# dibbelab/gficf

Hardware: AMD Instinct MI355X
Metric: jaccard_edges_per_sec (higher is better)
Workload: dtype int32

## Files before the change

### gficf_amd/csrc/knn.hip

```cpp
#include <cfloat>
#include <cstdlib>
#include <cstring>
#include <vector>

#include "common.h"
#include "knn_tiles.h"

namespace {

constexpr int KNN_MAX_D = 128;
constexpr int KNN_MAX_SPLIT = 16;

__host__ __device__ inline int knn_dpad(int d) { return (d + 3) & ~3; }

template <typename T>
__global__ __launch_bounds__(256) void k_knn_prepare(const T* __restrict__ X, int64_t n_rows, int d, int dpad, int64_t ld,
                                                     int metric, float* __restrict__ out, uint32_t* __restrict__ status) {
  const int64_t r = (int64_t)blockIdx.x * 256 + threadIdx.x;
  if (r >= n_rows) return;
  bool bad = false;
  float inv = 1.0f;
  bool scale = false;
  float mean = 0.0f;
  if (metric == GFICF_KNN_CORRELATION) {
// ... 71 lines not shown
  const int64_t e = (int64_t)blockIdx.x * 256 + threadIdx.x;
  if (e < n) v[e] = (int32_t)e;
}

constexpr int KNN_CELL_KEY_BITS = 20;
__global__ __launch_bounds__(256) void k_knn_sort_elems(const int32_t* __restrict__ pivot_of, const int32_t* __restrict__ coarse_of,
                                                        int64_t n, u64* __restrict__ kv) {
  const int64_t e = (int64_t)blockIdx.x * 256 + threadIdx.x;
  if (e < n) {
    const int32_t f = pivot_of[e];
    kv[e] = ((u64)(uint32_t)(((coarse_of[f - 1] - 1) << 12) | (f - 1)) << 32) | (u64)e;
  }
}

template <int METRIC>
__device__ inline float knn_bound_dist(const float* __restrict__ a, const float* __restrict__ b, int d) {
  float acc = 0.0f;
  for (int t = 0; t < d; ++t) {
    const float df = a[t] - b[t];
    acc = METRIC == GFICF_KNN_MANHATTAN ? acc + fabsf(df) : fmaf(df, df, acc);
  }
  return METRIC == GFICF_KNN_MANHATTAN ? acc : sqrtf(acc);
}

template <int METRIC>
__global__ __launch_bounds__(KNN_TC) void k_knn_tile_stats(const float* __restrict__ X, const int32_t* __restrict__ tile_n, int d, int dpad,
                                                           float* __restrict__ centers, float* __restrict__ radius) {
  __shared__ float s_c[KNN_MAX_D];
  __shared__ float s_r[KNN_TC / 64];
  const int64_t t = blockIdx.x, j0 = t * KNN_TC;
  const int n = tile_n[t];
  if (n <= 0) { if (threadIdx.x == 0) radius[t] = -1.0f; return; }
  for (int dim = threadIdx.x; dim < dpad; dim += KNN_TC) {
    float sum = 0.0f;
    for (int p = 0; p < n; ++p) sum += X[(j0 + p) * dpad + dim];
    const float c = sum / (float)n;
    s_c[dim] = c;
    centers[(int64_t)dim * gridDim.x + t] = c;
  }
  __syncthreads();
  float r = 0.0f;
  if ((int)threadIdx.x < n) r = knn_bound_dist<METRIC>(X + (j0 + threadIdx.x) * dpad, s_c, d);
#pragma unroll
  for (int w = 32; w >= 1; w >>= 1) r = fmaxf(r, __shfl_xor(r, w));
  if ((threadIdx.x & 63) == 0) s_r[threadIdx.x >> 6] = r;
  __syncthreads();
  if (threadIdx.x == 0) radius[t] = fmaxf(s_r[0], s_r[1]);
}

template <int METRIC>
__global__ __launch_bounds__(256) void k_knn_lb(const float* __restrict__ Q, const int32_t* __restrict__ qtile_n, int d, int dpad,
                                                const float* __restrict__ centers, const float* __restrict__ radius,
                                                const int32_t* __restrict__ tile_n, int kk, int64_t n_ct, float* __restrict__ lb,
                                                unsigned long long* __restrict__ counters) {
  extern __shared__ __attribute__((aligned(16))) float s_q[];
  __shared__ float s_u[4];
  const int64_t qt = blockIdx.x, q0 = qt * KNN_TQ;
  const int nq = qtile_n[qt];
  if (nq <= 0) return;
  for (int e = threadIdx.x; e < KNN_TQ * dpad; e += 256) {
    const int row = e / dpad, dim = e % dpad;
    s_q[dim * KNN_TQ + row] = row < nq ? Q[(q0 + row) * dpad + dim] : 0.0f;
  }
  __syncthreads();
  const int lane = threadIdx.x & 63, wave = threadIdx.x >> 6;
  const float key_abs_slack = (float)(d + 8) * 1.1920929e-7f;
  auto to_key = [key_abs_slack](float e, float slack_sign) {
    if (METRIC == GFICF_KNN_MANHATTAN) return e;
    if (METRIC == GFICF_KNN_EUCLIDEAN) return e * e * (1.0f + slack_sign * KNN_LB_SLACK);
    return 0.5f * e * e * (1.0f + slack_sign * KNN_LB_SLACK) + slack_sign * key_abs_slack;
  };
  float u = INFINITY;
  for (int64_t c = threadIdx.x; c < n_ct; c += 256) {
    const float r = radius[c];
    if (r < 0.0f) { lb[qt * n_ct + c] = INFINITY; continue; }
    float mn = INFINITY, mx = 0.0f;
    for (int g0 = 0; g0 < nq; g0 += 16) {
      float acc[16];
#pragma unroll
      for (int j = 0; j < 16; ++j) acc[j] = 0.0f;
      for (int t = 0; t < d; ++t) {
        const float cv = centers[(int64_t)t * n_ct + c];
        const float4* q4 = reinterpret_cast<const float4*>(s_q + t * KNN_TQ + g0);
#pragma unroll
        for (int j4 = 0; j4 < 4; ++j4) {
          const float4 q = q4[j4];
          const float qa[4] = {q.x, q.y, q.z, q.w};
#pragma unroll
          for (int j = 0; j < 4; ++j) {
            const float df = qa[j] - cv;
            acc[4 * j4 + j] = METRIC == GFICF_KNN_MANHATTAN ? acc[4 * j4 + j] + fabsf(df) : fmaf(df, df, acc[4 * j4 + j]);
          }
        }
      }
#pragma unroll
      for (int j = 0; j < 16; ++j) {
        if (g0 + j < nq) {
          const float e = METRIC == GFICF_KNN_MANHATTAN ? acc[j] : sqrtf(acc[j]);
          mn = fminf(mn, e); mx = fmaxf(mx, e);
        }
      }
    }
    float b = mn - r - KNN_LB_SLACK * (mn + r);
    b = b > 0.0f ? to_key(b, -1.0f) : 0.0f;
    lb[qt * n_ct + c] = b > 0.0f ? b : 0.0f;
    if (tile_n[c] >= kk) u = fminf(u, to_key((mx + r) * (1.0f + KNN_LB_SLACK), 1.0f));
  }
#pragma unroll
  for (int w = 32; w >= 1; w >>= 1) u = fminf(u, __shfl_xor(u, w));
  if (lane == 0) s_u[wave] = u;
  __syncthreads();
  const float U = fminf(fminf(s_u[0], s_u[1]), fminf(s_u[2], s_u[3]));
  int npr = 0, np = 0;
  for (int64_t c = threadIdx.x; c < n_ct; c += 256) {
    const float b = lb[qt * n_ct + c];
    if (b < INFINITY) { ++np; npr += b > U ? 1 : 0; }
  }
#pragma unroll
  for (int w = 32; w >= 1; w >>= 1) { npr += __shfl_xor(npr, w); np += __shfl_xor(np, w); }
  if (lane == 0) { atomicAdd(counters, (unsigned long long)npr); atomicAdd(counters + 1, (unsigned long long)np); }
}

__global__ void k_knn_choose(const unsigned long long* __restrict__ counters, uint32_t force, uint32_t* __restrict__ flag) {
  *flag = force ? 0u : (2ull * counters[0] < counters[1] ? 1u : 0u);
}

__global__ __launch_bounds__(256) void k_knn_cell_heads(const int32_t* __restrict__ keys, int64_t n, int64_t* __restrict__ flags) {
  const int64_t p = (int64_t)blockIdx.x * 256 + threadIdx.x;
  if (p > n) return;
  flags[p] = (p < n && (p == 0 || keys[p] != keys[p - 1])) ? 1 : 0;
}
__global__ __launch_bounds__(256) void k_knn_cell_starts(const int32_t* __restrict__ keys, const int64_t* __restrict__ rank, int64_t n,
                                                         int32_t* __restrict__ cstart) {
  const int64_t p = (int64_t)blockIdx.x * 256 + threadIdx.x;
  if (p > n) return;
  if (p == n) { cstart[rank[n]] = (int32_t)n; return; }
  if (p == 0 || keys[p] != keys[p - 1]) cstart[rank[p]] = (int32_t)p;
}
__global__ __launch_bounds__(1024) void k_knn_cell_offsets(const int32_t* __restrict__ cstart, const int64_t* __restrict__ n_cells_p, int T,
                                                           int32_t* __restrict__ pstart) {
  __shared__ int s_part[1024];
  __shared__ int s_total;
  const int n_cells = (int)*n_cells_p;
  const int per = (n_cells + 1023) / 1024;
  const int c0 = threadIdx.x * per;
  int sum = 0;
  for (int c = c0; c < c0 + per && c < n_cells; ++c) sum += (cstart[c + 1] - cstart[c] + T - 1) / T * T;
  s_part[threadIdx.x] = sum;
  __syncthreads();
  if (threadIdx.x == 0) {
    int run = 0;
    for (int t = 0; t < 1024; ++t) { const int v = s_part[t]; s_part[t] = run; run += v; }
    s_total = run;
  }
  __syncthreads();
  int run = s_part[threadIdx.x];
  for (int c = c0; c < c0 + per && c < n_cells; ++c) { pstart[c] = run; run += (cstart[c + 1] - cstart[c] + T - 1) / T * T; }
  if (threadIdx.x == 0) pstart[n_cells] = s_total;
}
__global__ __launch_bounds__(256) void k_knn_pad_scatter(const int32_t* __restrict__ keys, const int64_t* __restrict__ rank,
                                                         const int32_t* __restrict__ cstart, const int32_t* __restrict__ pstart,
                                                         const int32_t* __restrict__ perm, int64_t n, int nq4,
                                                         const float* __restrict__ src, float* __restrict__ dst, int32_t* __restrict__ perm_pad) {
  const int64_t e = (int64_t)blockIdx.x * 256 + threadIdx.x;
  if (e >= n * nq4) return;
  const int64_t p = e / nq4;
  const int q4 = (int)(e % nq4);
  const bool head = p == 0 || keys[p] != keys[p - 1];
  const int64_t c = rank[p] + (head ? 1 : 0) - 1;
  const int64_t pp = (int64_t)pstart[c] + (p - cstart[c]);
  const int32_t id = perm[p];
  reinterpret_cast<float4*>(dst)[pp * nq4 + q4] = reinterpret_cast<const float4*>(src)[(int64_t)id * nq4 + q4];
  if (q4 == 0) perm_pad[pp] = id;
// ... 1 lines not shown
__global__ __launch_bounds__(256) void k_knn_tile_counts(const int32_t* __restrict__ perm_pad, int64_t n_tiles, int T, int32_t* __restrict__ tile_n) {
  const int64_t t = (int64_t)blockIdx.x * 256 + threadIdx.x;
  if (t >= n_tiles) return;
  int n = 0;
  for (int r = 0; r < T; ++r) n += perm_pad[t * T + r] >= 0 ? 1 : 0;
  tile_n[t] = n;
}

int knn_split(const gficf_ctx* ctx, int64_t n_q, int64_t N) {
  const int64_t n_qt = gficf_ceil_div(n_q > 0 ? n_q : 1, KNN_TQ), n_ct = gficf_ceil_div(N > 0 ? N : 1, KNN_TC);
  int64_t S = gficf_ceil_div((int64_t)ctx->num_cus * 8, n_qt);
  if (S > n_ct / 8) S = n_ct / 8;
  if (S > KNN_MAX_SPLIT) S = KNN_MAX_SPLIT;
  if (S < 1) S = 1;
  if (const char* e = getenv("GFICF_KNN_SPLIT")) {
    const int v = atoi(e);
    if (v >= 1 && v <= KNN_MAX_SPLIT) S = v;
  }
  return (int)S;
}

constexpr int64_t KNN_PRUNE_MIN_N = 30000;
constexpr int64_t KNN_PRUNE_MAX_TILES = 8192;
bool knn_use_prune(int64_t N) {
  const int64_t n_ct = gficf_ceil_div(N > 0 ? N : 1, KNN_TC);
  if (n_ct < 2 || n_ct > KNN_PRUNE_MAX_TILES) return false;
  if (const char* e = getenv("GFICF_KNN_PRUNE")) return atoi(e) != 0;
  return N >= KNN_PRUNE_MIN_N;
}
inline int64_t knn_coarse(int64_t C) { return C / 16 > 2 ? C / 16 : 2; }

int64_t knn_pivots(int64_t N) {
  int64_t per = 256;
  if (const char* e = getenv("GFICF_KNN_PIVOT_CELL")) per = atoi(e) > 0 ? atoi(e) : per;
  int64_t c = gficf_ceil_div(N, per);
  return c < 2 ? 2 : c > 4096 ? 4096 : c;
}

int knn_check(int64_t N, int d, int k, int metric) {
  if (N < 0 || d < 0 || k < 0) GFICF_FAIL(GFICF_ERR_INVALID_ARG, "negative size");
  if (N > 0x7FFFFFFFll) GFICF_FAIL(GFICF_ERR_UNSUPPORTED, "N = %lld exceeds int32 ids", (long long)N);
  if (d > KNN_MAX_D) GFICF_FAIL(GFICF_ERR_UNSUPPORTED, "d = %d exceeds %d dimensions", d, KNN_MAX_D);
  if (k > GFICF_KNN_MAX_K) GFICF_FAIL(GFICF_ERR_UNSUPPORTED, "k = %d exceeds GFICF_KNN_MAX_K = %d", k, GFICF_KNN_MAX_K);
  if (k > N) GFICF_FAIL(GFICF_ERR_INVALID_ARG, "k = %d neighbours asked of N = %lld points", k, (long long)N);
  if (!gficf_knn_metric_ok(metric)) GFICF_FAIL(GFICF_ERR_INVALID_ARG, "unknown metric %d", metric);
  return GFICF_OK;
}

struct KnnPruneWs {
  int64_t C, xrows, qrows, n_ct, n_qt;
  float *pivots, *coarse, *xp, *qp, *centers, *radius, *lb;
  u64* apart;
  int32_t *pivot_of, *coarse_of, *key_tmp, *perm_sorted, *perm_x, *perm_q, *cstart, *pstart, *tile_n, *qtile_n;
  int64_t* rank;
  u64 *kv0, *kv1;
  int64_t* hist;
  u64* part;
  u64* part_plain;
  unsigned long long* counters;
  size_t total;
};

KnnPruneWs knn_prune_ws(char* base, int64_t n_q, int64_t N, int dpad, int k) {
  KnnPruneWs w{};
  gficf_carver cv{base};
  const int64_t C = knn_pivots(N);
  w.C = C;
  w.n_ct = gficf_ceil_div(N, KNN_TC) + (C < N ? C : N);
  w.n_qt = gficf_ceil_div(n_q, KNN_TQ) + (C < n_q ? C : n_q);
  w.xrows = w.n_ct * KNN_TC;
  w.qrows = w.n_qt * KNN_TQ;
  w.pivots = cv.take<float>((size_t)C * dpad);
  w.coarse = cv.take<float>((size_t)knn_coarse(C) * dpad);
  w.coarse_of = cv.take<int32_t>((size_t)C);
  w.xp = cv.take<float>((size_t)w.xrows * dpad);
  w.qp = cv.take<float>((size_t)w.qrows * dpad);
  w.centers = cv.take<float>((size_t)w.n_ct * dpad);
  w.radius = cv.take<float>((size_t)w.n_ct);
  w.lb = cv.take<float>((size_t)w.n_qt * w.n_ct);
  w.apart = cv.take<u64>((size_t)N);
  w.pivot_of = cv.take<int32_t>((size_t)N);
  w.key_tmp = cv.take<int32_t>((size_t)N);
  w.perm_sorted = cv.take<int32_t>((size_t)N);
  w.perm_x = cv.take<int32_t>((size_t)w.xrows);
  w.perm_q = cv.take<int32_t>((size_t)w.qrows);
  w.cstart = cv.take<int32_t>((size_t)(C + 2));
  w.pstart = cv.take<int32_t>((size_t)(C + 2));
  w.tile_n = cv.take<int32_t>((size_t)w.n_ct);
  w.qtile_n = cv.take<int32_t>((size_t)w.n_qt);
  w.rank = cv.take<int64_t>((size_t)(N + 1));
  w.kv0 = cv.take<u64>((size_t)N);
  w.kv1 = cv.take<u64>((size_t)N);
  w.hist = cv.take<int64_t>((size_t)gficf_radix_sort_hist_len(N, KNN_CELL_KEY_BITS));
  w.part = cv.take<u64>((size_t)w.qrows * (size_t)k);
  w.part_plain = cv.take<u64>((size_t)n_q * (size_t)KNN_MAX_SPLIT * (size_t)k);
  w.counters = cv.take<unsigned long long>(4);
  w.total = cv.total();
  return w;
}

}

extern "C" {

int gficf_knn_dpad(int d) { return (d < 0 || d > KNN_MAX_D) ? -1 : knn_dpad(d); }

int gficf_knn_prepare_device(gficf_ctx* ctx, const void* d_X, int x_is_f64, int64_t n_rows, int d, int64_t ld, int metric,
                             float* d_point_rows) {
  GFICF_CTX_ENTER(ctx);
  int rc = knn_check(n_rows, d, 0, metric);
  if (rc) return rc;
  if (n_rows == 0 || d == 0) return GFICF_OK;
  if (!d_X || !d_point_rows) GFICF_FAIL(GFICF_ERR_INVALID_ARG, "NULL device pointer");
  if (ld < n_rows) GFICF_FAIL(GFICF_ERR_INVALID_ARG, "ld = %lld < n_rows = %lld", (long long)ld, (long long)n_rows);
  const unsigned blocks = (unsigned)gficf_ceil_div(n_rows, 256);
  if (x_is_f64)
    hipLaunchKernelGGL(k_knn_prepare<double>, dim3(blocks), dim3(256), 0, ctx->stream, (const double*)d_X, n_rows, d, knn_dpad(d), ld, metric, d_point_rows, ctx->d_status);
  else
    hipLaunchKernelGGL(k_knn_prepare<float>, dim3(blocks), dim3(256), 0, ctx->stream, (const float*)d_X, n_rows, d, knn_dpad(d), ld, metric, d_point_rows, ctx->d_status);
  GFICF_HIP_CHECK(hipGetLastError());
  return GFICF_OK;
}

size_t gficf_knn_workspace_bytes(gficf_ctx* ctx, int64_t n_queries, int64_t N, int k) {
  if (!ctx || n_queries <= 0 || N <= 0 || k <= 0) return 256;
  const size_t plain = (size_t)n_queries * (size_t)KNN_MAX_SPLIT * (size_t)k * sizeof(u64) + 256;
  const size_t small = (size_t)n_queries * (size_t)knn_split(ctx, n_queries, N) * (size_t)k * sizeof(u64) + 256;
  const size_t pruned = gficf_ceil_div(N, KNN_TC) <= KNN_PRUNE_MAX_TILES ? knn_prune_ws(nullptr, n_queries, N, knn_dpad(KNN_MAX_D), k).total : 0;
  (void)plain;
  return small > pruned ? small : pruned;
}

int gficf_knn_search_device(gficf_ctx* ctx, const float* d_points, int64_t N, int d, int k, int metric, int64_t q_begin,
                            int64_t q_end, void* d_ws, size_t ws_bytes, int32_t* d_idx, float* d_dist, int64_t ld_out) {
  GFICF_CTX_ENTER(ctx);
  int rc = knn_check(N, d, k, metric);
  if (rc) return rc;
  if (q_begin < 0 || q_end < q_begin || q_end > N)
    GFICF_FAIL(GFICF_ERR_INVALID_ARG, "query range [%lld, %lld) outside [0, %lld]", (long long)q_begin, (long long)q_end, (long long)N);
  const int64_t n_q = q_end - q_begin;
  if (n_q == 0 || k == 0) return GFICF_OK;
  if (d == 0) GFICF_FAIL(GFICF_ERR_INVALID_ARG, "points have no dimensions");
  if (!d_points || !d_ws || !d_idx) GFICF_FAIL(GFICF_ERR_INVALID_ARG, "NULL device pointer");
  if (ld_out < n_q) GFICF_FAIL(GFICF_ERR_INVALID_ARG, "ld_out = %lld < number of queries %lld", (long long)ld_out, (long long)n_q);
  if (ws_bytes < gficf_knn_workspace_bytes(ctx, n_q, N, k)) GFICF_FAIL(GFICF_ERR_CAPACITY, "kNN workspace too small");
  metric = gficf_knn_search_metric(metric);
  const int dpad = knn_dpad(d);
  const unsigned mblocks = (unsigned)gficf_ceil_div(n_q, 256);
  KnnTileArgs a{};
  a.d = d; a.dpad = dpad; a.kk = k;

  if (!knn_use_prune(N)) {
    a.Q = d_points + q_begin * dpad; a.n_q = n_q; a.X = d_points; a.N = N;
    a.S = knn_split(ctx, n_q, N);
    a.part = (u64*)d_ws;
    rc = knn_launch_m<false>(ctx, metric, a);
    if (rc) return rc;
    hipLaunchKernelGGL(k_knn_merge, dim3(mblocks), dim3(256), 0, ctx->stream, a.part, n_q, a.S, k, metric, (const int32_t*)nullptr, d_idx, d_dist, ld_out, (const uint32_t*)nullptr, 0u);
    GFICF_HIP_CHECK(hipGetLastError());
    return GFICF_OK;
  }

  const KnnPruneWs w = knn_prune_ws((char*)d_ws, n_q, N, dpad, k);
  const int nq4 = dpad >> 2;
  const int64_t C = w.C;
  auto blocks_for = [](int64_t n) { return dim3((unsigned)gficf_ceil_div(n, 256)); };
  hipLaunchKernelGGL(k_knn_gather_rows, blocks_for(C * nq4), dim3(256), 0, ctx->stream, d_points, (const int32_t*)nullptr, C, nq4, N / C, w.pivots);
  KnnTileArgs as{};
  as.Q = d_points; as.n_q = N; as.X = w.pivots; as.N = C; as.d = d; as.dpad = dpad; as.kk = 1; as.S = 1; as.part = w.apart;
  rc = knn_launch_m<false>(ctx, metric, as);
  if (rc) return rc;
  hipLaunchKernelGGL(k_knn_merge, blocks_for(N), dim3(256), 0, ctx->stream, w.apart, N, 1, 1, metric, (const int32_t*)nullptr, w.pivot_of, (float*)nullptr, N, (const uint32_t*)nullptr, 0u);
  const int64_t Cc = knn_coarse(C);
  hipLaunchKernelGGL(k_knn_gather_rows, blocks_for(Cc * nq4), dim3(256), 0, ctx->stream, w.pivots, (const int32_t*)nullptr, Cc, nq4, C / Cc, w.coarse);
  KnnTileArgs ac{};
  ac.Q = w.pivots; ac.n_q = C; ac.X = w.coarse; ac.N = Cc; ac.d = d; ac.dpad = dpad; ac.kk = 1; ac.S = 1; ac.part = w.apart;
  rc = knn_launch_m<false>(ctx, metric, ac);
  if (rc) return rc;
  hipLaunchKernelGGL(k_knn_merge, blocks_for(C), dim3(256), 0, ctx->stream, w.apart, C, 1, 1, metric, (const int32_t*)nullptr, w.coarse_of, (float*)nullptr, C, (const uint32_t*)nullptr, 0u);
  GFICF_HIP_CHECK(hipMemsetAsync(w.xp, 0, sizeof(float) * (size_t)w.xrows * dpad, ctx->stream));
  GFICF_HIP_CHECK(hipMemsetAsync(w.qp, 0, sizeof(float) * (size_t)w.qrows * dpad, ctx->stream));
  GFICF_HIP_CHECK(hipMemsetAsync(w.perm_x, 0xFF, sizeof(int32_t) * (size_t)w.xrows, ctx->stream));
  GFICF_HIP_CHECK(hipMemsetAsync(w.perm_q, 0xFF, sizeof(int32_t) * (size_t)w.qrows, ctx->stream));
  auto layout = [&](int64_t first, int64_t n, int T, const float* src, float* dst, int32_t* perm_pad, int64_t n_tiles, int32_t* tile_n) -> int {
    hipLaunchKernelGGL(k_knn_sort_elems, blocks_for(n), dim3(256), 0, ctx->stream, w.pivot_of + first, w.coarse_of, n, w.kv0);
    int r = gficf_radix_sort_kv(ctx, w.kv0, w.kv1, w.hist, n, KNN_CELL_KEY_BITS, (uint32_t*)w.key_tmp, (uint32_t*)w.perm_sorted);
    if (r) return r;
    hipLaunchKernelGGL(k_knn_cell_heads, blocks_for(n + 1), dim3(256), 0, ctx->stream, w.key_tmp, n, w.rank);
    r = gficf_exclusive_scan_i64(ctx, w.rank, n + 1);
    if (r) return r;
    hipLaunchKernelGGL(k_knn_cell_starts, blocks_for(n + 1), dim3(256), 0, ctx->stream, w.key_tmp, w.rank, n, w.cstart);
    hipLaunchKernelGGL(k_knn_cell_offsets, dim3(1), dim3(1024), 0, ctx->stream, w.cstart, w.rank + n, T, w.pstart);
    hipLaunchKernelGGL(k_knn_pad_scatter, blocks_for(n * nq4), dim3(256), 0, ctx->stream, w.key_tmp, w.rank, w.cstart, w.pstart, w.perm_sorted, n, nq4,
                       src, dst, perm_pad);
    hipLaunchKernelGGL(k_knn_tile_counts, blocks_for(n_tiles), dim3(256), 0, ctx->stream, perm_pad, n_tiles, T, tile_n);
    GFICF_HIP_CHECK(hipGetLastError());
    return GFICF_OK;
  };
  rc = layout(0, N, KNN_TC, d_points, w.xp, w.perm_x, w.n_ct, w.tile_n);
  if (rc) return rc;
  rc = layout(q_begin, n_q, KNN_TQ, d_points + q_begin * dpad, w.qp, w.perm_q, w.n_qt, w.qtile_n);
  if (rc) return rc;
  GFICF_HIP_CHECK(hipMemsetAsync(w.counters, 0, 32, ctx->stream));
  const size_t lds_lb = (size_t)KNN_TQ * dpad * sizeof(float);
  switch (metric) {
    case GFICF_KNN_MANHATTAN:
      hipLaunchKernelGGL(k_knn_tile_stats<GFICF_KNN_MANHATTAN>, dim3((unsigned)w.n_ct), dim3(KNN_TC), 0, ctx->stream, w.xp, w.tile_n, d, dpad, w.centers, w.radius);
      hipLaunchKernelGGL(k_knn_lb<GFICF_KNN_MANHATTAN>, dim3((unsigned)w.n_qt), dim3(256), lds_lb, ctx->stream, w.qp, w.qtile_n, d, dpad, w.centers, w.radius, w.tile_n, k, w.n_ct, w.lb, w.counters);
      break;
    case GFICF_KNN_EUCLIDEAN:
      hipLaunchKernelGGL(k_knn_tile_stats<GFICF_KNN_EUCLIDEAN>, dim3((unsigned)w.n_ct), dim3(KNN_TC), 0, ctx->stream, w.xp, w.tile_n, d, dpad, w.centers, w.radius);
      hipLaunchKernelGGL(k_knn_lb<GFICF_KNN_EUCLIDEAN>, dim3((unsigned)w.n_qt), dim3(256), lds_lb, ctx->stream, w.qp, w.qtile_n, d, dpad, w.centers, w.radius, w.tile_n, k, w.n_ct, w.lb, w.counters);
      break;
    default:
      hipLaunchKernelGGL(k_knn_tile_stats<GFICF_KNN_COSINE>, dim3((unsigned)w.n_ct), dim3(KNN_TC), 0, ctx->stream, w.xp, w.tile_n, d, dpad, w.centers, w.radius);
      hipLaunchKernelGGL(k_knn_lb<GFICF_KNN_COSINE>, dim3((unsigned)w.n_qt), dim3(256), lds_lb, ctx->stream, w.qp, w.qtile_n, d, dpad, w.centers, w.radius, w.tile_n, k, w.n_ct, w.lb, w.counters);
      break;
  }
  GFICF_HIP_CHECK(hipGetLastError());
  uint32_t* const flag = (uint32_t*)(w.counters + 2);
  const char* fe = getenv("GFICF_KNN_PRUNE");
  hipLaunchKernelGGL(k_knn_choose, dim3(1), dim3(1), 0, ctx->stream, w.counters, (uint32_t)(fe && atoi(fe) != 0), flag);
  KnnTileArgs ap{};
  ap.Q = d_points + q_begin * dpad; ap.n_q = n_q; ap.X = d_points; ap.N = N; ap.d = d; ap.dpad = dpad; ap.kk = k;
  ap.S = knn_split(ctx, n_q, N); ap.part = w.part_plain; ap.gate = flag; ap.gate_want = 1u;
  rc = knn_launch_m<false>(ctx, metric, ap);
  if (rc) return rc;
  hipLaunchKernelGGL(k_knn_merge, dim3(mblocks), dim3(256), 0, ctx->stream, w.part_plain, n_q, ap.S, k, metric, (const int32_t*)nullptr, d_idx, d_dist, ld_out, (const uint32_t*)flag, 1u);
  a.Q = w.qp; a.n_q = w.qrows; a.X = w.xp; a.N = w.xrows; a.S = 1; a.part = w.part; a.perm_x = w.perm_x; a.lb = w.lb;
  a.tile_n = w.tile_n; a.qtile_n = w.qtile_n; a.gate = flag; a.gate_want = 0u;
  rc = knn_launch_m<true>(ctx, metric, a);
  if (rc) return rc;
  hipLaunchKernelGGL(k_knn_merge, blocks_for(w.qrows), dim3(256), 0, ctx->stream, w.part, w.qrows, 1, k, metric, (const int32_t*)w.perm_q, d_idx, d_dist, ld_out, (const uint32_t*)flag, 0u);
  GFICF_HIP_CHECK(hipGetLastError());
  return GFICF_OK;
}

int gficf_knn_pivot_order_device(gficf_ctx* ctx, const float* d_points, int64_t N, int d, int metric, void* d_ws, size_t ws_bytes,
                                 int32_t* d_order) {
  GFICF_CTX_ENTER(ctx);
  int rc = knn_check(N, d, 1, metric);
  if (rc) return rc;
  if (N == 0) return GFICF_OK;
  if (d == 0) GFICF_FAIL(GFICF_ERR_INVALID_ARG, "points have no dimensions");
  if (!d_points || !d_ws || !d_order) GFICF_FAIL(GFICF_ERR_INVALID_ARG, "NULL device pointer");
  if (ws_bytes < gficf_knn_workspace_bytes(ctx, N, N, 1)) GFICF_FAIL(GFICF_ERR_CAPACITY, "kNN workspace too small");
  metric = gficf_knn_search_metric(metric);
  auto blocks_for = [](int64_t n) { return dim3((unsigned)gficf_ceil_div(n, 256)); };
  if (gficf_ceil_div(N, KNN_TC) > KNN_PRUNE_MAX_TILES || knn_pivots(N) < 2) {
    hipLaunchKernelGGL(k_knn_iota, blocks_for(N), dim3(256), 0, ctx->stream, d_order, N);
    GFICF_HIP_CHECK(hipGetLastError());
    return GFICF_OK;
  }
  const int dpad = knn_dpad(d);
  const KnnPruneWs w = knn_prune_ws((char*)d_ws, N, N, dpad, 1);
  const int nq4 = dpad >> 2;
  const int64_t C = w.C;
  hipLaunchKernelGGL(k_knn_gather_rows, blocks_for(C * nq4), dim3(256), 0, ctx->stream, d_points, (const int32_t*)nullptr, C, nq4, N / C, w.pivots);
  KnnTileArgs as{};
  as.Q = d_points; as.n_q = N; as.X = w.pivots; as.N = C; as.d = d; as.dpad = dpad; as.kk = 1; as.S = 1; as.part = w.apart;
  rc = knn_launch_m<false>(ctx, metric, as);
  if (rc) return rc;
  hipLaunchKernelGGL(k_knn_merge, blocks_for(N), dim3(256), 0, ctx->stream, w.apart, N, 1, 1, metric, (const int32_t*)nullptr, w.pivot_of, (float*)nullptr, N, (const uint32_t*)nullptr, 0u);
  const int64_t Cc = knn_coarse(C);
  hipLaunchKernelGGL(k_knn_gather_rows, blocks_for(Cc * nq4), dim3(256), 0, ctx->stream, w.pivots, (const int32_t*)nullptr, Cc, nq4, C / Cc, w.coarse);
  KnnTileArgs ac{};
  ac.Q = w.pivots; ac.n_q = C; ac.X = w.coarse; ac.N = Cc; ac.d = d; ac.dpad = dpad; ac.kk = 1; ac.S = 1; ac.part = w.apart;
  rc = knn_launch_m<false>(ctx, metric, ac);
  if (rc) return rc;
  hipLaunchKernelGGL(k_knn_merge, blocks_for(C), dim3(256), 0, ctx->stream, w.apart, C, 1, 1, metric, (const int32_t*)nullptr, w.coarse_of, (float*)nullptr, C, (const uint32_t*)nullptr, 0u);
  hipLaunchKernelGGL(k_knn_sort_elems, blocks_for(N), dim3(256), 0, ctx->stream, w.pivot_of, w.coarse_of, N, w.kv0);
  GFICF_HIP_CHECK(hipGetLastError());
  return gficf_radix_sort_kv(ctx, w.kv0, w.kv1, w.hist, N, KNN_CELL_KEY_BITS, (uint32_t*)w.key_tmp, (uint32_t*)d_order);
}

int gficf_knn_host(gficf_ctx* ctx, const double* X, int64_t N, int d, int64_t ld, int k, int metric, int32_t* idx, double* dist) {
  GFICF_CTX_ENTER(ctx);
  int rc = knn_check(N, d, k, metric);
  if (rc) return rc;
  if (N == 0 || k == 0) return GFICF_OK;
  if (d == 0) GFICF_FAIL(GFICF_ERR_INVALID_ARG, "points have no dimensions");
  if (!X || !idx) GFICF_FAIL(GFICF_ERR_INVALID_ARG, "NULL host pointer");
  if (ld < N) GFICF_FAIL(GFICF_ERR_INVALID_ARG, "ld = %lld < N = %lld", (long long)ld, (long long)N);
// ... 32 lines not shown
```

### gficf_amd/csrc/knn_tiles.h

```cpp
#pragma once

#include <atomic>
#include <type_traits>

#include "common.h"

namespace {

constexpr int KNN_TC = 128;
constexpr int KNN_DK = 16;
constexpr int KNN_THREADS = 256;
constexpr int KNN_RQ = 4;
constexpr int KNN_TQ = 16 * KNN_RQ;

typedef unsigned long long u64;

__device__ inline uint32_t f32_sortable(float f) {
  const uint32_t u = __float_as_uint(f);
  return u ^ ((uint32_t)((int32_t)u >> 31) | 0x80000000u);
}
__device__ inline float sortable_f32(uint32_t s) {
  return __uint_as_float(s ^ (((s >> 31) - 1u) | 0x80000000u));
}

typedef __attribute__((address_space(3))) volatile u64 knn_lds_u64;

template <int KL>
__device__ __noinline__ float knn_row_insert(uint32_t list_addr, int kk, float d0, float d1, float d2, float d3, float d4, float d5,
                                             float d6, float d7, float tau, bool live, uint32_t j0, int tid,
                                             const int32_t* __restrict__ perm) {
  knn_lds_u64* const list = (knn_lds_u64*)(size_t)list_addr;
  const float dv[8] = {d0, d1, d2, d3, d4, d5, d6, d7};
  const int tx = tid & 15;
  uint32_t pass = 0;
  if (live) {
#pragma unroll
    for (int s = 0; s < 8; ++s) pass |= (dv[s] <= tau) ? 1u << s : 0u;
  }
  for (;;) {
    const u64 m = __ballot(pass != 0);
    if (m == 0) break;
    const uint32_t gm = (uint32_t)(m >> (tid & 48)) & 0xFFFFu;
    const int leader = __ffs(gm) - 1;
    uint32_t khi = 0, klo = 0;
    if (pass != 0 && tx == leader) {
      const int s = __ffs(pass) - 1;
      pass &= pass - 1;
      float h = dv[0];
#pragma unroll
      for (int t = 1; t < 8; ++t) h = s == t ? dv[t] : h;
      khi = f32_sortable(h);
      klo = j0 + (uint32_t)((s < 4 ? 0 : 64) + tx * 4 + (s & 3));
      if (perm) klo = (uint32_t)perm[klo];
    }
    const int src = ((tid & 48) | (leader & 15)) << 2;
    khi = (uint32_t)__builtin_amdgcn_ds_bpermute(src, (int)khi);
    klo = (uint32_t)__builtin_amdgcn_ds_bpermute(src, (int)klo);
    if (leader >= 0) {
      const u64 key = ((u64)khi << 32) | (u64)klo;
      u64 nw[KL / 16];
#pragma unroll
      for (int e = 0; e < KL / 16; ++e) {
        const int pos = e * 16 + tx;
        const u64 cur = list[pos];
        const u64 prev = pos > 0 ? list[pos - 1] : 0ull;
        nw[e] = cur <= key ? cur : (prev <= key ? key : prev);
// ... 41 lines not shown
      } else {
        acc[r][s] = __builtin_elementwise_fma(ar, b[s], acc[r][s]);
      }
    }
  }
}

template <int EPL>
__device__ __forceinline__ void knn_reg_insert(u64 (&lst)[EPL], u64 key) {
  const u64 last = lst[EPL - 1];
  const uint32_t plo = (uint32_t)__builtin_amdgcn_update_dpp(0, (int)(uint32_t)last, 0x111, 0xf, 0xf, true);
  const uint32_t phi = (uint32_t)__builtin_amdgcn_update_dpp(0, (int)(uint32_t)(last >> 32), 0x111, 0xf, 0xf, true);
  u64 prev = ((u64)phi << 32) | (u64)plo;
#pragma unroll
  for (int h = 0; h < EPL; ++h) {
    const u64 cur = lst[h];
    lst[h] = cur <= key ? cur : (prev <= key ? key : prev);
    prev = cur;
  }
}

struct KnnTileArgs {
  const float* Q;
  int64_t n_q;
  const float* X;
  int64_t N;
  int d, dpad, kk, S;
  u64* part;
  const int32_t* perm_x;
  const float* lb;
  const int32_t* tile_n;
  const int32_t* qtile_n;
  const uint32_t* gate;
  uint32_t gate_want;
};

template <int METRIC, int KL, int RQ, bool PRUNE>
__global__ __launch_bounds__(KNN_THREADS, 2) void k_knn_tiles(const KnnTileArgs A) {
  constexpr int TQ = 16 * RQ;
  if (A.gate != nullptr && *A.gate != A.gate_want) return;
  extern __shared__ __attribute__((aligned(16))) unsigned char smem[];
  const int d = A.d, dpad = A.dpad, kk = A.kk, S = A.S;
  const int64_t N = A.N;
  float* const sA = reinterpret_cast<float*>(smem);
  float* const sB = sA + (size_t)dpad * TQ;
  constexpr bool REGL = KL <= 64;
  constexpr int EPL = KL / 16;
  u64* const sKey = reinterpret_cast<u64*>(sB + 2 * KNN_DK * KNN_TC);
  float* const sLb = reinterpret_cast<float*>(sKey + (REGL ? 0 : TQ * KL));
  const uint32_t key_addr = (uint32_t)(size_t)(__attribute__((address_space(3))) unsigned char*)(unsigned char*)sKey;
  __shared__ float s_wtau[2][KNN_THREADS / 64];

  const int tid = threadIdx.x, tx = tid & 15, ty = tid >> 4, lane = tid & 63, wave = tid >> 6;
  const int qt = blockIdx.x / S, sp = blockIdx.x % S;
  const int64_t q0 = (int64_t)qt * TQ;
  const int nq_live = (PRUNE && A.qtile_n) ? A.qtile_n[qt] : (A.n_q - q0 < TQ ? (int)(A.n_q - q0) : TQ);
  if (nq_live <= 0) return;
  const int64_t n_ct = gficf_ceil_div(N, KNN_TC);
  const int64_t ct0 = PRUNE ? 0 : n_ct * sp / S, ct1 = PRUNE ? n_ct : n_ct * (sp + 1) / S;
  const int nq4 = dpad >> 2;
  const int nch = (d + KNN_DK - 1) / KNN_DK;
  const float4* const X4 = reinterpret_cast<const float4*>(A.X);
  const float4* const Q4 = reinterpret_cast<const float4*>(A.Q);

  if (!REGL)
    for (int e = tid; e < TQ * KL; e += KNN_THREADS) sKey[e] = ~0ull;
  u64 lst[RQ][REGL ? EPL : 1];
#pragma unroll
  for (int r = 0; r < RQ; ++r)
#pragma unroll
    for (int h = 0; h < (REGL ? EPL : 1); ++h) lst[r][h] = ~0ull;
  for (int f = tid; f < TQ * nq4; f += KNN_THREADS) {
    const int row = f & (TQ - 1), quad = f / TQ;
    const int64_t q = q0 + row;
    const float4 v = q < A.n_q ? Q4[q * nq4 + quad] : make_float4(0.f, 0.f, 0.f, 0.f);
    float* o = sA + (size_t)(quad * 4) * TQ + row;
    o[0] = v.x; o[TQ] = v.y; o[2 * TQ] = v.z; o[3 * TQ] = v.w;
  }
  if (PRUNE) {
    for (int64_t e = tid; e < n_ct; e += KNN_THREADS) sLb[e] = A.lb[(int64_t)qt * n_ct + e];
    if (tid < 2 * (KNN_THREADS / 64)) s_wtau[tid / (KNN_THREADS / 64)][tid % (KNN_THREADS / 64)] = INFINITY;
  }

  const int row_l = tid & (KNN_TC - 1), quad0 = tid >> 7;
  float* const st0 = sB + (size_t)(quad0 * 4) * KNN_TC + row_l;
  auto load_chunk = [&](int64_t ct, int c, float4 (&v)[2]) {
    const int64_t j = ct * KNN_TC + row_l;
    const int q4 = c * (KNN_DK / 4) + quad0;
    const float4* src = X4 + j * nq4 + q4;
    v[0] = (j < N && q4 < nq4) ? src[0] : make_float4(0.f, 0.f, 0.f, 0.f);
    v[1] = (j < N && q4 + 2 < nq4) ? src[2] : make_float4(0.f, 0.f, 0.f, 0.f);
  };
  auto store_chunk = [&](int buf, const float4 (&v)[2]) {
    float* o = st0 + (size_t)buf * KNN_DK * KNN_TC;
    o[0] = v[0].x; o[KNN_TC] = v[0].y; o[2 * KNN_TC] = v[0].z; o[3 * KNN_TC] = v[0].w;
    o += 8 * KNN_TC;
    o[0] = v[1].x; o[KNN_TC] = v[1].y; o[2 * KNN_TC] = v[1].z; o[3 * KNN_TC] = v[1].w;
  };
  auto select_tile = [&](int64_t skip, int par) -> int64_t {
    float best = INFINITY;
    int bi = -1;
    for (int e = lane; e < (int)n_ct; e += 64) {
      const float v = sLb[e];
      if (e != (int)skip && v < best) { best = v; bi = e; }
    }
#pragma unroll
    for (int w = 32; w >= 1; w >>= 1) {
      const float ov = __shfl_xor(best, w);
      const int oi = __shfl_xor(bi, w);
      if (ov < best || (ov == best && oi >= 0 && (bi < 0 || oi < bi))) { best = ov; bi = oi; }
    }
    float tmax = s_wtau[par][0];
#pragma unroll
    for (int w = 1; w < KNN_THREADS / 64; ++w) tmax = fmaxf(tmax, s_wtau[par][w]);
    return (bi >= 0 && best <= tmax) ? (int64_t)bi : -1;
  };

  knn_f2 acc[RQ][4];
#pragma unroll
  for (int r = 0; r < RQ; ++r)
#pragma unroll
    for (int s = 0; s < 4; ++s) acc[r][s] = knn_f2{0.0f, 0.0f};

  float tau[RQ];
#pragma unroll
  for (int r = 0; r < RQ; ++r) tau[r] = INFINITY;

  __syncthreads();
  int64_t cur = PRUNE ? select_tile(-1, 0) : (ct0 < ct1 ? ct0 : -1);
  float4 pre[2];
  if (cur >= 0) { load_chunk(cur, 0, pre); store_chunk(0, pre); }
  __syncthreads();

  int buf = 0, tile_no = 0;
  while (cur >= 0) {
    if (PRUNE && tid == 0) sLb[cur] = INFINITY;
    int64_t nxt = -1;
    for (int c = 0; c < nch; ++c) {
      bool have_next;
      if (c + 1 < nch) {
        load_chunk(cur, c + 1, pre);
        have_next = true;
      } else {
        nxt = PRUNE ? select_tile(cur, (tile_no + 1) & 1) : (cur + 1 < ct1 ? cur + 1 : -1);
        have_next = nxt >= 0;
        if (have_next) load_chunk(nxt, 0, pre);
      }
      const float* const pa = sA + (size_t)(c * KNN_DK) * TQ + ty * 4;
      const float* const pb = sB + (size_t)buf * KNN_DK * KNN_TC + tx * 4;
      const int nd = d - c * KNN_DK < KNN_DK ? d - c * KNN_DK : KNN_DK;
      {
        const int np = (nd + 1) >> 1;
        KnnOperands oa, ob;
        knn_read<RQ>(oa, pa, pb);
#pragma unroll 1
        for (int t = 0; t < np; ++t) {
          knn_read<RQ>(ob, pa + (2 * t + 1) * TQ, pb + (2 * t + 1) * KNN_TC);
          knn_dim<METRIC, RQ>(acc, oa);
          if (t + 1 < np) knn_read<RQ>(oa, pa + (2 * t + 2) * TQ, pb + (2 * t + 2) * KNN_TC);
          knn_dim<METRIC, RQ>(acc, ob);
        }
      }
      if (c == nch - 1) {
        const int64_t j0 = cur * KNN_TC;
        const int nvalid = (PRUNE && A.tile_n) ? A.tile_n[cur] : (N - j0 < KNN_TC ? (int)(N - j0) : KNN_TC);
        auto epilogue = [&](auto rag_tag) {
          constexpr bool RAG = decltype(rag_tag)::value;
#pragma unroll
// ... 64 lines not shown
                th = (uint32_t)__shfl((int)th, (kk - 1) / EPL, 16);
                tau[r] = th == 0xFFFFFFFFu ? INFINITY : sortable_f32(th);
              } else {
                tau[r] = knn_row_insert<KL>(key_addr + (uint32_t)(row * KL * 8), kk, dv[0], dv[1], dv[2], dv[3], dv[4], dv[5], dv[6],
                                            dv[7], tau[r], live, (uint32_t)j0, tid, PRUNE ? A.perm_x : (const int32_t*)nullptr);
              }
            }
#pragma unroll
            for (int s = 0; s < 4; ++s) acc[r][s] = knn_f2{0.0f, 0.0f};
          }
        };
        if (nvalid < KNN_TC) epilogue(std::true_type{});
        else epilogue(std::false_type{});
        if (PRUNE) {
          float tm = 0.0f;
#pragma unroll
          for (int r = 0; r < RQ; ++r)
            if ((r < 4 ? 0 : 64) + ty * 4 + (r & 3) < nq_live) tm = fmaxf(tm, tau[r]);
          tm = fmaxf(tm, __shfl_xor(tm, 16));
          tm = fmaxf(tm, __shfl_xor(tm, 32));
          if (lane == 0) s_wtau[tile_no & 1][wave] = tm;
        }
      }
      if (have_next) store_chunk(buf ^ 1, pre);
      __syncthreads();
      buf ^= 1;
    }
    cur = nxt;
    ++tile_no;
  }

  if (REGL) {
#pragma unroll
    for (int r = 0; r < RQ; ++r) {
      const int64_t q = q0 + (r < 4 ? 0 : 64) + ty * 4 + (r & 3);
#pragma unroll
      for (int h = 0; h < (REGL ? EPL : 1); ++h) {
        const int e = EPL * tx + h;
        if (q < A.n_q && e < kk) A.part[(q * S + sp) * kk + e] = lst[r][h];
      }
    }
  } else {
    for (int e = tid; e < TQ * kk; e += KNN_THREADS) {
      const int row = e / kk, t = e % kk;
      const int64_t q = q0 + row;
      if (q < A.n_q) A.part[(q * S + sp) * kk + t] = sKey[row * KL + t];
    }
  }
}

template <int METRIC, int KL, bool PRUNE>
int knn_launch(gficf_ctx* ctx, const KnnTileArgs& a) {
  const int64_t n_ct = gficf_ceil_div(a.N, KNN_TC);
  const size_t lds = (size_t)a.dpad * KNN_TQ * 4 + 2 * KNN_DK * KNN_TC * 4 + (KL > 64 ? (size_t)KNN_TQ * KL * 8 : 0) + (PRUNE ? (size_t)n_ct * 4 : 0);
  static std::atomic<bool> attr_set[64];
  if (!attr_set[ctx->device & 63]) {
    GFICF_HIP_CHECK(hipFuncSetAttribute((const void*)k_knn_tiles<METRIC, KL, KNN_RQ, PRUNE>, hipFuncAttributeMaxDynamicSharedMemorySize, 160 * 1024 - 64));
    attr_set[ctx->device & 63] = true;
  }
  const int64_t blocks = gficf_ceil_div(a.n_q, KNN_TQ) * a.S;
  hipLaunchKernelGGL((k_knn_tiles<METRIC, KL, KNN_RQ, PRUNE>), dim3((unsigned)blocks), dim3(KNN_THREADS), lds, ctx->stream, a);
  GFICF_HIP_CHECK(hipGetLastError());
  return GFICF_OK;
}

template <int METRIC, bool PRUNE>
int knn_launch_k(gficf_ctx* ctx, const KnnTileArgs& a) {
  if (a.kk <= 32) return knn_launch<METRIC, 32, PRUNE>(ctx, a);
  if (a.kk <= 64) return knn_launch<METRIC, 64, PRUNE>(ctx, a);
  return knn_launch<METRIC, 128, PRUNE>(ctx, a);
}

template <bool PRUNE>
int knn_launch_m(gficf_ctx* ctx, int metric, const KnnTileArgs& a) {
  switch (metric) {
    case GFICF_KNN_MANHATTAN: return knn_launch_k<GFICF_KNN_MANHATTAN, PRUNE>(ctx, a);
    case GFICF_KNN_EUCLIDEAN: return knn_launch_k<GFICF_KNN_EUCLIDEAN, PRUNE>(ctx, a);
    default: return knn_launch_k<GFICF_KNN_COSINE, PRUNE>(ctx, a);
  }
}

}
```

Before: 62.95 billion.

## Cache reachable tile list in LDS and schedule query tiles by reach

```diff
diff --git a/gficf_amd/csrc/knn.hip b/gficf_amd/csrc/knn.hip
--- a/gficf_amd/csrc/knn.hip
+++ b/gficf_amd/csrc/knn.hip
@@ -147,7 +147,7 @@
 __global__ __launch_bounds__(256) void k_knn_lb(const float* __restrict__ Q, const int32_t* __restrict__ qtile_n, int d, int dpad,
                                                 const float* __restrict__ centers, const float* __restrict__ radius,
                                                 const int32_t* __restrict__ tile_n, int kk, int64_t n_ct, float* __restrict__ lb,
-                                                unsigned long long* __restrict__ counters) {
+                                                unsigned long long* __restrict__ counters, int32_t* __restrict__ reach) {
   extern __shared__ __attribute__((aligned(16))) float s_q[];
   __shared__ float s_u[4];
   const int64_t qt = blockIdx.x, q0 = qt * KNN_TQ;
@@ -213,7 +213,25 @@
   }
 #pragma unroll
   for (int w = 32; w >= 1; w >>= 1) { npr += __shfl_xor(npr, w); np += __shfl_xor(np, w); }
-  if (lane == 0) { atomicAdd(counters, (unsigned long long)npr); atomicAdd(counters + 1, (unsigned long long)np); }
+  if (lane == 0) {
+    atomicAdd(counters, (unsigned long long)npr); atomicAdd(counters + 1, (unsigned long long)np);
+    atomicAdd(reach + qt, np - npr);
+  }
+}
+
+__global__ __launch_bounds__(256) void k_knn_order(const int32_t* __restrict__ reach, int n, int32_t* __restrict__ order) {
+  const int i = blockIdx.x * 4 + (threadIdx.x >> 6), lane = threadIdx.x & 63;
+  const int mine = i < n ? reach[i] : -1;
+  int rank = 0;
+  for (int j = lane * 4; j < n; j += 256) {
+    const int4 v4 = *reinterpret_cast<const int4*>(reach + j);
+    const int v[4] = {v4.x, v4.y, v4.z, v4.w};
+#pragma unroll
+    for (int e = 0; e < 4; ++e) rank += (j + e < n && (v[e] > mine || (v[e] == mine && j + e < i))) ? 1 : 0;
+  }
+#pragma unroll
+  for (int w = 32; w >= 1; w >>= 1) rank += __shfl_xor(rank, w);
+  if (i < n && lane == 0) order[rank] = i;
 }
 
 __global__ void k_knn_choose(const unsigned long long* __restrict__ counters, uint32_t force, uint32_t* __restrict__ flag) {
@@ -321,6 +339,7 @@
   float *pivots, *coarse, *xp, *qp, *centers, *radius, *lb;
   u64* apart;
   int32_t *pivot_of, *coarse_of, *key_tmp, *perm_sorted, *perm_x, *perm_q, *cstart, *pstart, *tile_n, *qtile_n;
+  int32_t *reach, *order;
   int64_t* rank;
   u64 *kv0, *kv1;
   int64_t* hist;
@@ -356,14 +375,16 @@
   w.cstart = cv.take<int32_t>((size_t)(C + 2));
   w.pstart = cv.take<int32_t>((size_t)(C + 2));
   w.tile_n = cv.take<int32_t>((size_t)w.n_ct);
-  w.qtile_n = cv.take<int32_t>((size_t)w.n_qt);
+  w.qtile_n = cv.take<int32_t>(2 * (size_t)w.n_qt);
+  w.order = w.qtile_n + (base ? w.n_qt : 0);
   w.rank = cv.take<int64_t>((size_t)(N + 1));
   w.kv0 = cv.take<u64>((size_t)N);
   w.kv1 = cv.take<u64>((size_t)N);
   w.hist = cv.take<int64_t>((size_t)gficf_radix_sort_hist_len(N, KNN_CELL_KEY_BITS));
   w.part = cv.take<u64>((size_t)w.qrows * (size_t)k);
   w.part_plain = cv.take<u64>((size_t)n_q * (size_t)KNN_MAX_SPLIT * (size_t)k);
-  w.counters = cv.take<unsigned long long>(4);
+  w.counters = cv.take<unsigned long long>(4 + (size_t)(w.n_qt + 3) / 4 * 2);
+  w.reach = (int32_t*)(w.counters + (base ? 4 : 0));
   w.total = cv.total();
   return w;
 }
@@ -470,20 +491,20 @@
   if (rc) return rc;
   rc = layout(q_begin, n_q, KNN_TQ, d_points + q_begin * dpad, w.qp, w.perm_q, w.n_qt, w.qtile_n);
   if (rc) return rc;
-  GFICF_HIP_CHECK(hipMemsetAsync(w.counters, 0, 32, ctx->stream));
+  GFICF_HIP_CHECK(hipMemsetAsync(w.counters, 0, 32 + sizeof(int32_t) * (size_t)w.n_qt, ctx->stream));
   const size_t lds_lb = (size_t)KNN_TQ * dpad * sizeof(float);
   switch (metric) {
     case GFICF_KNN_MANHATTAN:
       hipLaunchKernelGGL(k_knn_tile_stats<GFICF_KNN_MANHATTAN>, dim3((unsigned)w.n_ct), dim3(KNN_TC), 0, ctx->stream, w.xp, w.tile_n, d, dpad, w.centers, w.radius);
-      hipLaunchKernelGGL(k_knn_lb<GFICF_KNN_MANHATTAN>, dim3((unsigned)w.n_qt), dim3(256), lds_lb, ctx->stream, w.qp, w.qtile_n, d, dpad, w.centers, w.radius, w.tile_n, k, w.n_ct, w.lb, w.counters);
+      hipLaunchKernelGGL(k_knn_lb<GFICF_KNN_MANHATTAN>, dim3((unsigned)w.n_qt), dim3(256), lds_lb, ctx->stream, w.qp, w.qtile_n, d, dpad, w.centers, w.radius, w.tile_n, k, w.n_ct, w.lb, w.counters, w.reach);
       break;
     case GFICF_KNN_EUCLIDEAN:
       hipLaunchKernelGGL(k_knn_tile_stats<GFICF_KNN_EUCLIDEAN>, dim3((unsigned)w.n_ct), dim3(KNN_TC), 0, ctx->stream, w.xp, w.tile_n, d, dpad, w.centers, w.radius);
-      hipLaunchKernelGGL(k_knn_lb<GFICF_KNN_EUCLIDEAN>, dim3((unsigned)w.n_qt), dim3(256), lds_lb, ctx->stream, w.qp, w.qtile_n, d, dpad, w.centers, w.radius, w.tile_n, k, w.n_ct, w.lb, w.counters);
+      hipLaunchKernelGGL(k_knn_lb<GFICF_KNN_EUCLIDEAN>, dim3((unsigned)w.n_qt), dim3(256), lds_lb, ctx->stream, w.qp, w.qtile_n, d, dpad, w.centers, w.radius, w.tile_n, k, w.n_ct, w.lb, w.counters, w.reach);
       break;
     default:
       hipLaunchKernelGGL(k_knn_tile_stats<GFICF_KNN_COSINE>, dim3((unsigned)w.n_ct), dim3(KNN_TC), 0, ctx->stream, w.xp, w.tile_n, d, dpad, w.centers, w.radius);
-      hipLaunchKernelGGL(k_knn_lb<GFICF_KNN_COSINE>, dim3((unsigned)w.n_qt), dim3(256), lds_lb, ctx->stream, w.qp, w.qtile_n, d, dpad, w.centers, w.radius, w.tile_n, k, w.n_ct, w.lb, w.counters);
+      hipLaunchKernelGGL(k_knn_lb<GFICF_KNN_COSINE>, dim3((unsigned)w.n_qt), dim3(256), lds_lb, ctx->stream, w.qp, w.qtile_n, d, dpad, w.centers, w.radius, w.tile_n, k, w.n_ct, w.lb, w.counters, w.reach);
       break;
   }
   GFICF_HIP_CHECK(hipGetLastError());
@@ -498,6 +519,7 @@
   hipLaunchKernelGGL(k_knn_merge, dim3(mblocks), dim3(256), 0, ctx->stream, w.part_plain, n_q, ap.S, k, metric, (const int32_t*)nullptr, d_idx, d_dist, ld_out, (const uint32_t*)flag, 1u);
   a.Q = w.qp; a.n_q = w.qrows; a.X = w.xp; a.N = w.xrows; a.S = 1; a.part = w.part; a.perm_x = w.perm_x; a.lb = w.lb;
   a.tile_n = w.tile_n; a.qtile_n = w.qtile_n; a.gate = flag; a.gate_want = 0u;
+  hipLaunchKernelGGL(k_knn_order, dim3((unsigned)gficf_ceil_div(w.n_qt, 4)), dim3(256), 0, ctx->stream, w.reach, (int)w.n_qt, w.order);
   rc = knn_launch_m<true>(ctx, metric, a);
   if (rc) return rc;
   hipLaunchKernelGGL(k_knn_merge, blocks_for(w.qrows), dim3(256), 0, ctx->stream, w.part, w.qrows, 1, k, metric, (const int32_t*)w.perm_q, d_idx, d_dist, ld_out, (const uint32_t*)flag, 0u);
diff --git a/gficf_amd/csrc/knn_tiles.h b/gficf_amd/csrc/knn_tiles.h
--- a/gficf_amd/csrc/knn_tiles.h
+++ b/gficf_amd/csrc/knn_tiles.h
@@ -12,6 +12,18 @@
 constexpr int KNN_THREADS = 256;
 constexpr int KNN_RQ = 4;
 constexpr int KNN_TQ = 16 * KNN_RQ;
+constexpr int KNN_REACH = 256;
+constexpr size_t KNN_LDS_MAX = 160 * 1024 - 64;
+struct KnnLds {
+  size_t bytes;
+  int reach_cap;
+};
+__host__ __device__ inline KnnLds knn_lds_bytes(int dpad, int KL, int64_t n_ct, bool prune) {
+  const size_t base = (size_t)dpad * KNN_TQ * 4 + 2 * KNN_DK * KNN_TC * 4 + (KL > 64 ? (size_t)KNN_TQ * KL * 8 : 0);
+  if (!prune) return {base, 0};
+  const size_t bounds = (size_t)((n_ct + 1) & ~(int64_t)1) * 4, list = 2 * (size_t)KNN_REACH * 8;
+  return base + bounds + list <= KNN_LDS_MAX ? KnnLds{base + bounds + list, KNN_REACH} : KnnLds{base + (size_t)n_ct * 4, 0};
+}
 
 typedef unsigned long long u64;
 
@@ -159,11 +171,13 @@
   __shared__ float s_wtau[2][KNN_THREADS / 64];
 
   const int tid = threadIdx.x, tx = tid & 15, ty = tid >> 4, lane = tid & 63, wave = tid >> 6;
-  const int qt = blockIdx.x / S, sp = blockIdx.x % S;
+  const int qt = (PRUNE && A.qtile_n) ? A.qtile_n[gridDim.x + blockIdx.x] : blockIdx.x / S, sp = blockIdx.x % S;
   const int64_t q0 = (int64_t)qt * TQ;
   const int nq_live = (PRUNE && A.qtile_n) ? A.qtile_n[qt] : (A.n_q - q0 < TQ ? (int)(A.n_q - q0) : TQ);
   if (nq_live <= 0) return;
   const int64_t n_ct = gficf_ceil_div(N, KNN_TC);
+  [[maybe_unused]] u64* const s_reach = reinterpret_cast<u64*>(sLb + ((n_ct + 1) & ~(int64_t)1));
+  [[maybe_unused]] const int reach_cap = PRUNE ? knn_lds_bytes(dpad, KL, n_ct, true).reach_cap : 0;
   const int64_t ct0 = PRUNE ? 0 : n_ct * sp / S, ct1 = PRUNE ? n_ct : n_ct * (sp + 1) / S;
   const int nq4 = dpad >> 2;
   const int nch = (d + KNN_DK - 1) / KNN_DK;
@@ -204,23 +218,56 @@
     o += 8 * KNN_TC;
     o[0] = v[1].x; o[KNN_TC] = v[1].y; o[2 * KNN_TC] = v[1].z; o[3 * KNN_TC] = v[1].w;
   };
+  int reach_n = -1;
   auto select_tile = [&](int64_t skip, int par) -> int64_t {
-    float best = INFINITY;
-    int bi = -1;
-    for (int e = lane; e < (int)n_ct; e += 64) {
-      const float v = sLb[e];
-      if (e != (int)skip && v < best) { best = v; bi = e; }
-    }
-#pragma unroll
-    for (int w = 32; w >= 1; w >>= 1) {
-      const float ov = __shfl_xor(best, w);
-      const int oi = __shfl_xor(bi, w);
-      if (ov < best || (ov == best && oi >= 0 && (bi < 0 || oi < bi))) { best = ov; bi = oi; }
-    }
     float tmax = s_wtau[par][0];
 #pragma unroll
     for (int w = 1; w < KNN_THREADS / 64; ++w) tmax = fmaxf(tmax, s_wtau[par][w]);
-    return (bi >= 0 && best <= tmax) ? (int64_t)bi : -1;
+    const u64 below = (1ull << lane) - 1ull;
+    u64 best = ~0ull;
+    int cnt = 0;
+    if (reach_n < 0) {
+      for (int e0 = 0; e0 < (int)n_ct; e0 += 64) {
+        const int e = e0 + lane;
+        const float v = e < (int)n_ct ? sLb[e] : INFINITY;
+        const bool in = e != (int)skip && v < INFINITY && v <= tmax;
+        const u64 key = ((u64)__float_as_uint(v) << 32) | (u64)(uint32_t)e;
+        best = (in && key < best) ? key : best;
+        const u64 m = __ballot(in);
+        const int pos = cnt + __popcll(m & below);
+        if (in && pos < reach_cap) s_reach[par * KNN_REACH + pos] = key;
+        cnt += __popcll(m);
+      }
+      if (cnt <= reach_cap) reach_n = cnt;
+    } else {
+      for (int e0 = 0; e0 < reach_n; e0 += 64) {
+        const u64 key = e0 + lane < reach_n ? s_reach[(par ^ 1) * KNN_REACH + e0 + lane] : ~0ull;
+        const bool in = key != ~0ull && (uint32_t)key != (uint32_t)(int)skip && __uint_as_float((uint32_t)(key >> 32)) <= tmax;
+        best = (in && key < best) ? key : best;
+        const u64 m = __ballot(in);
+        if (in) s_reach[par * KNN_REACH + cnt + __popcll(m & below)] = key;
+        cnt += __popcll(m);
+      }
+      reach_n = cnt;
+    }
+    auto dpp_min = [&](auto ctrl) {
+      const uint32_t lo = (uint32_t)__builtin_amdgcn_update_dpp(0, (int)(uint32_t)best, decltype(ctrl)::value, 0xf, 0xf, false);
+      const uint32_t hi = (uint32_t)__builtin_amdgcn_update_dpp(0, (int)(uint32_t)(best >> 32), decltype(ctrl)::value, 0xf, 0xf, false);
+      const u64 o = ((u64)hi << 32) | (u64)lo;
+      best = o < best ? o : best;
+    };
+    dpp_min(std::integral_constant<int, 0xB1>{});
+    dpp_min(std::integral_constant<int, 0x4E>{});
+    dpp_min(std::integral_constant<int, 0x141>{});
+    dpp_min(std::integral_constant<int, 0x140>{});
+    u64 wbest = ~0ull;
+#pragma unroll
+    for (int row = 0; row < 4; ++row) {
+      const u64 o = ((u64)(uint32_t)__builtin_amdgcn_readlane((int)(uint32_t)(best >> 32), row * 16) << 32) |
+                    (u64)(uint32_t)__builtin_amdgcn_readlane((int)(uint32_t)best, row * 16);
+      wbest = o < wbest ? o : wbest;
+    }
+    return wbest != ~0ull ? (int64_t)(uint32_t)wbest : -1;
   };
 
   knn_f2 acc[RQ][4];
@@ -391,10 +438,10 @@
 template <int METRIC, int KL, bool PRUNE>
 int knn_launch(gficf_ctx* ctx, const KnnTileArgs& a) {
   const int64_t n_ct = gficf_ceil_div(a.N, KNN_TC);
-  const size_t lds = (size_t)a.dpad * KNN_TQ * 4 + 2 * KNN_DK * KNN_TC * 4 + (KL > 64 ? (size_t)KNN_TQ * KL * 8 : 0) + (PRUNE ? (size_t)n_ct * 4 : 0);
+  const size_t lds = knn_lds_bytes(a.dpad, KL, n_ct, PRUNE).bytes;
   static std::atomic<bool> attr_set[64];
   if (!attr_set[ctx->device & 63]) {
-    GFICF_HIP_CHECK(hipFuncSetAttribute((const void*)k_knn_tiles<METRIC, KL, KNN_RQ, PRUNE>, hipFuncAttributeMaxDynamicSharedMemorySize, 160 * 1024 - 64));
+    GFICF_HIP_CHECK(hipFuncSetAttribute((const void*)k_knn_tiles<METRIC, KL, KNN_RQ, PRUNE>, hipFuncAttributeMaxDynamicSharedMemorySize, (int)KNN_LDS_MAX));
     attr_set[ctx->device & 63] = true;
   }
   const int64_t blocks = gficf_ceil_div(a.n_q, KNN_TQ) * a.S;
```

Result: no change. 62.93 billion (-0.0%).
